# fudan-zvg/NeRF-LiDAR

Measured on AMD Instinct MI355X. Metric: LiDAR rays/sec @128 samples/ray, 8x256 MLP; depth L1 vs reference, higher is better.
Workload: dtype f32 (sampling, hash grid) + split-bf16 x3 MFMA (density/semantic/intensity) + bf16 MFMA (view MLP); 1 GPU; C2: nuScenes 32-beam sweep, 32x1024 rays per sweep, samples (64,64,128), 8x256 NerfMLP + semantic + intensity heads, full-size fp32 hash tables; azimuth_columns_total=1024, parallelism=azimuth-sector x1, hip_graph_replay=False, weights=seeded synthetic (white-noise tables, x1500 density gain), sweep_origins=moving: step i renders sweep i mod 64 (pre-uploaded ray batches), gather_bytes_per_ray=1347584

## Files before the change

nerf-lidar_amd/csrc/nlr_sample.hip:

```cpp
#include "nlr_kernels.h"

struct ResampleParams {
    const float *prev_sdist;
    const float *prev_weights;
    uint32_t n_prev;
    float dilation;
    float anneal, pad;
    uint32_t S;
    const float *u;
    const float *jitter;
    float max_jitter;
    const float *near, *far;
    float lam, lam1, c_fwd, inv_exp;
    uint32_t N;
    float *sdist, *tdist;
};

__device__ __forceinline__ float nlr_warp_fwd(float x, float lam, float lam1, float c_fwd) {
    return c_fwd * (powf((x * 2.0f) / lam1 + 1.0f, lam) - 1.0f);
}
__device__ __forceinline__ float nlr_warp_inv(float y, float lam, float lam1, float inv_exp) {
    return ((powf(((y * lam) / lam1 + 1.0f) + NLR_EPS, inv_exp) - 1.0f) * lam1) / 2.0f;
}

__global__ void __launch_bounds__(64) nlr_resample_kernel(ResampleParams P) {
    extern __shared__ __align__(16) float lds[];
    const uint32_t ray = blockIdx.x;
    const int lane = threadIdx.x;
    const uint32_t n = P.n_prev;
    const bool dilate = (n > 0) && (P.dilation > 0.0f);

    float *tt;
    float *ww;
    uint32_t m;
    float *scratch;

    if (n == 0) {
        tt = lds;
        ww = lds + 2;
        if (lane == 0) {
            tt[0] = 0.0f;
            tt[1] = 1.0f;
            ww[0] = 1.0f;
        }
        m = 1;
        scratch = lds + 4;
    } else {
        float *t = lds;
        float *p = t + (n + 1);
        const float *ps = P.prev_sdist + (size_t)ray * (n + 1);
        const float *pw = P.prev_weights + (size_t)ray * n;
        for (uint32_t i = lane; i <= n; i += 64) t[i] = ps[i];
        for (uint32_t i = lane; i < n; i += 64) p[i] = pw[i];
        __syncthreads();
        if (!dilate) {
            tt = t;
            ww = p;
            m = n;
            scratch = p + n;
        } else {
            float *U = p + n;
            float *W = U + (3 * n + 2);
            float *Mx = W + 3 * n;
            const float d = P.dilation;
            for (uint32_t j = lane; j < n; j += 64) p[j] = p[j] / fmaxf(t[j + 1] - t[j], NLR_EPS);
            auto count = [&](uint32_t len, auto pred) {
                uint32_t lo = 0, hi = len;
                while (lo < hi) {
                    const uint32_t mid = (lo + hi) >> 1;
                    if (pred(mid)) lo = mid + 1; else hi = mid;
                }
                return lo;
            };
            for (uint32_t i = lane; i <= 3 * n; i += 64) {
                float v;
                uint32_t r;
                if (i <= n) {
                    v = t[i];
                    r = i + count(n, [&](uint32_t q) { return (t[q] - d) < v; }) + count(n, [&](uint32_t q) { return (t[q + 1] + d) < v; });
                } else if (i <= 2 * n) {
                    const uint32_t o = i - (n + 1);
                    v = t[o] - d;
                    r = o + count(n + 1, [&](uint32_t q) { return t[q] <= v; }) + count(n, [&](uint32_t q) { return (t[q + 1] + d) < v; });
                } else {
                    const uint32_t o = i - (2 * n + 1);
                    v = t[o + 1] + d;
                    r = o + count(n + 1, [&](uint32_t q) { return t[q] <= v; }) + count(n, [&](uint32_t q) { return (t[q] - d) <= v; });
                }
                U[r] = fminf(fmaxf(v, 0.0f), 1.0f);
            }
            uint32_t LV = 1;
            while ((2u << (LV - 1)) <= n) ++LV;
            __syncthreads();
            for (uint32_t l = 1; l < LV; ++l) {
                const float *src = l == 1 ? p : Mx + (size_t)(l - 2) * n;
                float *dst = Mx + (size_t)(l - 1) * n;
                const uint32_t h2 = 1u << (l - 1);
                for (uint32_t j = lane; j < n; j += 64) {
                    const uint32_t j2 = j + h2 < n ? j + h2 : n - 1;
                    dst[j] = fmaxf(src[j], src[j2]);
                }
                __syncthreads();
            }
            float part = 0.0f;
            for (uint32_t k = lane; k < 3 * n; k += 64) {
                const float tk = U[k];
                const uint32_t j1 = count(n, [&](uint32_t q) { return (t[q] - d) <= tk; });
                const uint32_t j0 = count(n, [&](uint32_t q) { return (t[q + 1] + d) <= tk; });
                float best = 0.0f;
                if (j0 < j1) {
                    const uint32_t len = j1 - j0, l = 31u - (uint32_t)__clz((int)len);
                    const float *row = l == 0 ? p : Mx + (size_t)(l - 1) * n;
                    best = fmaxf(best, fmaxf(row[j0], row[j1 - (1u << l)]));
                }
                const float wk = best * (U[k + 1] - tk);
                W[k] = wk;
                part += wk;
            }
            const float tot = fmaxf(nlr_wave_sum(part), NLR_EPS);
            __syncthreads();
            for (uint32_t k = lane; k < 3 * n; k += 64) W[k] = W[k] / tot;
            __syncthreads();
            tt = U + 1;
            ww = W + 1;
            m = 3 * n - 2;
            scratch = Mx + (size_t)(LV - 1) * n;
        }
    }
    __syncthreads();

    float *cw = scratch;
    float *cen = cw + (m + 1);
    float mx = -INFINITY;
    for (uint32_t k = lane; k < m; k += 64) {
        const float lg = (tt[k + 1] > tt[k]) ? P.anneal * logf(ww[k] + P.pad) : -INFINITY;
        cw[k + 1] = lg;
        mx = fmaxf(mx, lg);
    }
    mx = nlr_wave_max(mx);
    float se = 0.0f;
    for (uint32_t k = lane; k < m; k += 64) {
        const float e = expf(cw[k + 1] - mx);
        cw[k + 1] = e;
        se += e;
    }
    se = nlr_wave_sum(se);
    __syncthreads();
    {
        const uint32_t per = (m + 63) / 64;
        const uint32_t b0 = lane * per;
        float run = 0.0f;
        for (uint32_t i = 0; i < per; ++i) {
            const uint32_t k = b0 + i;
            if (k < m) run += cw[k + 1] / se;
        }
        const float incl = nlr_wave_incl_scan_add(run, lane);
        float base = incl - run;
        float prevmax = nlr_wave_incl_scan_max(incl, lane);
        prevmax = __shfl_up(prevmax, 1, 64);
        if (lane == 0) prevmax = 0.0f;
        __syncthreads();
        float acc = base;
        float hi = prevmax;
        for (uint32_t i = 0; i < per; ++i) {
            const uint32_t k = b0 + i;
            if (k < m) {
                acc += cw[k + 1] / se;
                hi = fmaxf(hi, acc);
                cw[k + 1] = (k + 1 == m) ? 1.0f : fminf(hi, 1.0f);
            }
        }
        if (lane == 0) cw[0] = 0.0f;
    }
    __syncthreads();

    const float jit = P.jitter ? P.jitter[ray] * P.max_jitter : 0.0f;
    for (uint32_t k = lane; k < P.S; k += 64) {
        const float u = P.jitter ? P.u[k] + jit : P.u[k];
        uint32_t lo = 0, hi = m + 1;
        while (lo < hi) {
            const uint32_t mid = (lo + hi) >> 1;
            if (cw[mid] <= u) lo = mid + 1; else hi = mid;
        }
        const uint32_t i0 = lo > 0 ? (lo - 1 > m ? m : lo - 1) : 0;
        const uint32_t i1 = lo > m ? m : lo;
        const float x0 = cw[i0], x1 = cw[i1];
        float off = (u - x0) / (x1 - x0);
        if (off != off) off = 0.0f;
        off = fminf(fmaxf(off, 0.0f), 1.0f);
        cen[k] = tt[i0] + off * (tt[i1] - tt[i0]);
    }
    __syncthreads();

    const float nearv = P.near[ray], farv = P.far[ray];
    const float s_near = nlr_warp_fwd(nearv, P.lam, P.lam1, P.c_fwd);
    const float s_far = nlr_warp_fwd(farv, P.lam, P.lam1, P.c_fwd);
    float *so = P.sdist + (size_t)ray * (P.S + 1);
    float *to = P.tdist ? P.tdist + (size_t)ray * (P.S + 1) : nullptr;
    for (uint32_t k = lane; k <= P.S; k += 64) {
        float s;
        if (k == 0) {
            const float mid0 = (cen[1] + cen[0]) / 2.0f;
            s = fmaxf(2.0f * cen[0] - mid0, 0.0f);
        } else if (k == P.S) {
            const float midl = (cen[P.S - 1] + cen[P.S - 2]) / 2.0f;
            s = fminf(2.0f * cen[P.S - 1] - midl, 1.0f);
        } else {
            s = (cen[k] + cen[k - 1]) / 2.0f;
        }
        so[k] = s;
        if (to) to[k] = nlr_warp_inv(s * s_far + (1.0f - s) * s_near, P.lam, P.lam1, P.inv_exp);
    }
}

static void linspace_f32(float start, float end, uint32_t n, float *out) {
    if (n == 1) {
        out[0] = start;
        return;
    }
    const float step = (end - start) / (float)(n - 1);
    const uint32_t half = n / 2;
    for (uint32_t i = 0; i < n; ++i) out[i] = i < half ? start + step * (float)i : end - step * (float)(n - 1 - i);
}

extern "C" void nlr_sample_u(uint32_t n, int rand, float *u_host, float *max_jitter) {
    const double eps = (double)NLR_EPS;
    if (!rand) {
        const double pad = 1.0 / (2.0 * n);
        linspace_f32((float)pad, (float)(1.0 - pad - eps), n, u_host);
        if (max_jitter) *max_jitter = 0.0f;
    } else {
        const double u_max = eps + (1.0 - eps) / n;
        linspace_f32(0.0f, (float)(1.0 - u_max), n, u_host);
        if (max_jitter) *max_jitter = (float)((1.0 - u_max) / (n - 1) - eps);
    }
}

int nlr_launch_resample(const float *prev_sdist, const float *prev_weights, uint32_t n_prev, float dilation, float anneal,
                        float pad, uint32_t S, const float *u_dev, const float *jitter, float max_jitter, const float *near,
                        const float *far, float lam, uint32_t N, float *sdist, float *tdist, hipStream_t st) {
    NLR_CHECK_ARG(S >= 2, "num_samples must be > 1, is %u", S);
    NLR_CHECK_ARG(S <= 1024 && n_prev <= 512, "resample: S=%u / n_prev=%u beyond the LDS budget", S, n_prev);
    NLR_CHECK_ARG((n_prev == 0) || (prev_sdist && prev_weights), "resample: previous level tensors are NULL");
    ResampleParams P;
    memset(&P, 0, sizeof(P));
    P.prev_sdist = prev_sdist;
    P.prev_weights = prev_weights;
    P.n_prev = n_prev;
    P.dilation = dilation;
    P.anneal = anneal;
    P.pad = pad;
    P.S = S;
    P.u = u_dev;
    P.jitter = jitter;
    P.max_jitter = max_jitter;
    P.near = near;
    P.far = far;
    P.lam = lam;
    P.lam1 = fabsf(lam - 1.0f);
    P.c_fwd = (float)(fabs((double)lam - 1.0) / (double)lam);
    P.inv_exp = (float)(1.0 / (double)lam);
    P.N = N;
    P.sdist = sdist;
    P.tdist = tdist;
    const bool dilate = n_prev > 0 && dilation > 0.0f;
    size_t fl;
    uint32_t m;
    if (n_prev == 0) {
        fl = 4;
        m = 1;
    } else if (!dilate) {
        fl = 2 * (size_t)n_prev + 1;
        m = n_prev;
    } else {
        uint32_t lv = 1;
        while ((2u << (lv - 1)) <= n_prev) ++lv;
        fl = 2 * (size_t)n_prev + 1 + (3 * (size_t)n_prev + 2) + 3 * (size_t)n_prev + (size_t)(lv - 1) * n_prev;
        m = 3 * n_prev - 2;
    }
    fl += (m + 1) + S + 8;
    const size_t lds_bytes = fl * sizeof(float);
    NLR_CHECK_ARG(lds_bytes <= 64 * 1024, "resample: LDS need %zu B > 64 KiB", lds_bytes);
    hipLaunchKernelGGL(nlr_resample_kernel, dim3(N), dim3(64), lds_bytes, st, P);
    NLR_LAUNCH_CHECK("nlr_resample_kernel");
    return NLR_OK;
}

extern "C" int nlr_resample_level(const float *prev_sdist, const float *prev_weights, uint32_t n_prev, float dilation,
                                  float anneal, float resample_padding, uint32_t num_samples, const float *rand_jitter,
                                  const float *near, const float *far, float power_lambda, uint32_t N, float *sdist,
                                  float *tdist, void *stream) {
    NLR_CHECK_ARG(near && far && sdist, "resample_level: NULL tensor");
    if (N == 0) return NLR_OK;
    NLR_CHECK_ARG(num_samples >= 2 && num_samples <= 1024, "num_samples must be in [2,1024], is %u", num_samples);
    hipStream_t st = (hipStream_t)stream;
    float uh[1024], mj = 0.0f;
    nlr_sample_u(num_samples, rand_jitter != nullptr, uh, &mj);
    float *u_dev = nullptr;
    NLR_HIP(hipMallocAsync((void **)&u_dev, num_samples * sizeof(float), st));
    NLR_HIP(hipMemcpyAsync(u_dev, uh, num_samples * sizeof(float), hipMemcpyHostToDevice, st));
    NLR_HIP(hipStreamSynchronize(st));
    int rc = nlr_launch_resample(prev_sdist, prev_weights, n_prev, dilation, anneal, resample_padding, num_samples, u_dev,
                                 rand_jitter, mj, near, far, power_lambda, N, sdist, tdist, st);
    (void)hipFreeAsync(u_dev, st);
    return rc;
}
```

Measured before the change: 5.173 million rays/s.

## Replace per-element binary searches with chunked merge-style searches in resample kernel

The dilation merge-rank and max-query phases now give each lane a contiguous chunk and search two sorted lists at once. The first element of a chunk is searched in full, and the following elements narrow the bounds using the neighbouring lane's result via shuffles. Shifted boundary arrays are precomputed into LDS, the inverse-CDF sampling uses the same chunked search, and the first pass skips the softmax/scan when weights are uniform. It also computes the near/far warp in two lanes and broadcasts the result. The cost targeted is the many full-length LDS binary searches per element, at the price of more complex indexing, extra LDS scratch and load imbalance across lanes.

Result: faster. 5.346 million rays/s (median of 6 runs) (+3.3%).

```diff
diff --git a/nerf-lidar_amd/csrc/nlr_sample.hip b/nerf-lidar_amd/csrc/nlr_sample.hip
--- a/nerf-lidar_amd/csrc/nlr_sample.hip
+++ b/nerf-lidar_amd/csrc/nlr_sample.hip
@@ -23,6 +23,19 @@
     return ((powf(((y * lam) / lam1 + 1.0f) + NLR_EPS, inv_exp) - 1.0f) * lam1) / 2.0f;
 }
 
+__device__ __forceinline__ void nlr_count2(const float *l1, uint32_t &lo1, uint32_t hi1, bool eq1, const float *l2, uint32_t &lo2,
+                                           uint32_t hi2, bool eq2, float v) {
+    while (lo1 < hi1 || lo2 < hi2) {
+        const uint32_t m1 = (lo1 + hi1) >> 1, m2 = (lo2 + hi2) >> 1;
+        const float x1 = l1[m1], x2 = l2[m2];
+        const bool b1 = (x1 < v) | ((x1 == v) & eq1), b2 = (x2 < v) | ((x2 == v) & eq2);
+        lo1 = (b1 & (lo1 < hi1)) ? m1 + 1 : lo1;
+        hi1 = b1 ? hi1 : m1;
+        lo2 = (b2 & (lo2 < hi2)) ? m2 + 1 : lo2;
+        hi2 = b2 ? hi2 : m2;
+    }
+}
+
 __global__ void __launch_bounds__(64) nlr_resample_kernel(ResampleParams P) {
     extern __shared__ __align__(16) float lds[];
     const uint32_t ray = blockIdx.x;
@@ -34,6 +47,7 @@
     float *ww;
     uint32_t m;
     float *scratch;
+    bool uniform = false;
 
     if (n == 0) {
         tt = lds;
@@ -45,6 +59,8 @@
         }
         m = 1;
         scratch = lds + 4;
+        const float lg = P.anneal * logf(1.0f + P.pad);
+        uniform = (lg - lg) == 0.0f;
     } else {
         float *t = lds;
         float *p = t + (n + 1);
@@ -63,34 +79,43 @@
             float *W = U + (3 * n + 2);
             float *Mx = W + 3 * n;
             const float d = P.dilation;
-            for (uint32_t j = lane; j < n; j += 64) p[j] = p[j] / fmaxf(t[j + 1] - t[j], NLR_EPS);
-            auto count = [&](uint32_t len, auto pred) {
-                uint32_t lo = 0, hi = len;
-                while (lo < hi) {
-                    const uint32_t mid = (lo + hi) >> 1;
-                    if (pred(mid)) lo = mid + 1; else hi = mid;
-                }
-                return lo;
-            };
-            for (uint32_t i = lane; i <= 3 * n; i += 64) {
-                float v;
-                uint32_t r;
-                if (i <= n) {
-                    v = t[i];
-                    r = i + count(n, [&](uint32_t q) { return (t[q] - d) < v; }) + count(n, [&](uint32_t q) { return (t[q + 1] + d) < v; });
-                } else if (i <= 2 * n) {
-                    const uint32_t o = i - (n + 1);
-                    v = t[o] - d;
-                    r = o + count(n + 1, [&](uint32_t q) { return t[q] <= v; }) + count(n, [&](uint32_t q) { return (t[q + 1] + d) < v; });
-                } else {
-                    const uint32_t o = i - (2 * n + 1);
-                    v = t[o + 1] + d;
-                    r = o + count(n + 1, [&](uint32_t q) { return t[q] <= v; }) + count(n, [&](uint32_t q) { return (t[q] - d) <= v; });
-                }
-                U[r] = fminf(fmaxf(v, 0.0f), 1.0f);
-            }
             uint32_t LV = 1;
             while ((2u << (LV - 1)) <= n) ++LV;
+            float *t0 = Mx + (size_t)(LV - 1) * n;
+            float *t1 = t0 + n;
+            for (uint32_t j = lane; j < n; j += 64) {
+                const float a = t[j], b = t[j + 1];
+                p[j] = p[j] / fmaxf(b - a, NLR_EPS);
+                t0[j] = a - d;
+                t1[j] = b + d;
+            }
+            __syncthreads();
+            {
+                uint32_t per = (3 * n + 1 + 63) / 64;
+                while ((n + per) / per + 2 * ((n + per - 1) / per) > 64) ++per;
+                const uint32_t LA = (n + per) / per, LB = (n + per - 1) / per;
+                const uint32_t kind = (uint32_t)lane < LA ? 0u : ((uint32_t)lane < LA + LB ? 1u : 2u);
+                const float *own = kind == 0 ? t : (kind == 1 ? t0 : t1);
+                const float *l1 = kind == 0 ? t0 : t, *l2 = kind == 2 ? t0 : t1;
+                const uint32_t own_len = kind == 0 ? n + 1 : n, len1 = kind == 0 ? n : n + 1, len2 = n;
+                const bool eq1 = kind != 0, eq2 = kind == 2;
+                const uint32_t first_lane = kind == 0 ? 0u : (kind == 1 ? LA : LA + LB);
+                const uint32_t o0 = ((uint32_t)lane - first_lane) * per;
+                const uint32_t o1 = o0 + per < own_len ? o0 + per : own_len;
+                const bool act = o0 < own_len;
+                uint32_t c1 = 0, c2 = 0;
+                float v = act ? own[o0] : 0.0f;
+                nlr_count2(l1, c1, act ? len1 : 0u, eq1, l2, c2, act ? len2 : 0u, eq2, v);
+                const uint32_t n1 = __shfl_down(c1, 1, 64), n2 = __shfl_down(c2, 1, 64);
+                const bool next_same = ((uint32_t)lane + 1 - first_lane) * per < own_len && lane < 63;
+                const uint32_t up1 = next_same ? n1 : len1, up2 = next_same ? n2 : len2;
+                if (act) U[o0 + c1 + c2] = fminf(fmaxf(v, 0.0f), 1.0f);
+                for (uint32_t o = o0 + 1; o < o1; ++o) {
+                    v = own[o];
+                    nlr_count2(l1, c1, up1, eq1, l2, c2, up2, eq2, v);
+                    U[o + c1 + c2] = fminf(fmaxf(v, 0.0f), 1.0f);
+                }
+            }
             __syncthreads();
             for (uint32_t l = 1; l < LV; ++l) {
                 const float *src = l == 1 ? p : Mx + (size_t)(l - 2) * n;
@@ -102,21 +127,36 @@
                 }
                 __syncthreads();
             }
+            {
+                const uint32_t per = (3 * n + 63) / 64;
+                const uint32_t k0 = (uint32_t)lane * per, k1 = k0 + per < 3 * n ? k0 + per : 3 * n;
+                float tk = 0.0f;
+                const auto emit = [&](uint32_t k, uint32_t j0, uint32_t j1) {
+                    float best = 0.0f;
+                    if (j0 < j1) {
+                        const uint32_t len = j1 - j0, l = 31u - (uint32_t)__clz((int)len);
+                        const float *row = l == 0 ? p : Mx + (size_t)(l - 1) * n;
+                        best = fmaxf(best, fmaxf(row[j0], row[j1 - (1u << l)]));
+                    }
+                    W[k] = best * (U[k + 1] - tk);
+                };
+                const bool act = k0 < 3 * n;
+                uint32_t j1 = 0, j0 = 0;
+                if (act) tk = U[k0];
+                nlr_count2(t0, j1, act ? n : 0u, true, t1, j0, act ? n : 0u, true, tk);
+                const uint32_t nj1 = __shfl_down(j1, 1, 64), nj0 = __shfl_down(j0, 1, 64);
+                const bool next_act = ((uint32_t)lane + 1) * per < 3 * n && lane < 63;
+                const uint32_t up1 = next_act ? nj1 : n, up0 = next_act ? nj0 : n;
+                if (act) emit(k0, j0, j1);
+                for (uint32_t k = k0 + 1; k < k1; ++k) {
+                    tk = U[k];
+                    nlr_count2(t0, j1, up1, true, t1, j0, up0, true, tk);
+                    emit(k, j0, j1);
+                }
+            }
+            __syncthreads();
             float part = 0.0f;
-            for (uint32_t k = lane; k < 3 * n; k += 64) {
-                const float tk = U[k];
-                const uint32_t j1 = count(n, [&](uint32_t q) { return (t[q] - d) <= tk; });
-                const uint32_t j0 = count(n, [&](uint32_t q) { return (t[q + 1] + d) <= tk; });
-                float best = 0.0f;
-                if (j0 < j1) {
-                    const uint32_t len = j1 - j0, l = 31u - (uint32_t)__clz((int)len);
-                    const float *row = l == 0 ? p : Mx + (size_t)(l - 1) * n;
-                    best = fmaxf(best, fmaxf(row[j0], row[j1 - (1u << l)]));
-                }
-                const float wk = best * (U[k + 1] - tk);
-                W[k] = wk;
-                part += wk;
-            }
+            for (uint32_t k = lane; k < 3 * n; k += 64) part += W[k];
             const float tot = fmaxf(nlr_wave_sum(part), NLR_EPS);
             __syncthreads();
             for (uint32_t k = lane; k < 3 * n; k += 64) W[k] = W[k] / tot;
@@ -131,70 +171,93 @@
 
     float *cw = scratch;
     float *cen = cw + (m + 1);
-    float mx = -INFINITY;
-    for (uint32_t k = lane; k < m; k += 64) {
-        const float lg = (tt[k + 1] > tt[k]) ? P.anneal * logf(ww[k] + P.pad) : -INFINITY;
-        cw[k + 1] = lg;
-        mx = fmaxf(mx, lg);
-    }
-    mx = nlr_wave_max(mx);
-    float se = 0.0f;
-    for (uint32_t k = lane; k < m; k += 64) {
-        const float e = expf(cw[k + 1] - mx);
-        cw[k + 1] = e;
-        se += e;
-    }
-    se = nlr_wave_sum(se);
+    if (uniform) {
+        if (lane == 0) {
+            cw[0] = 0.0f;
+            cw[1] = 1.0f;
+        }
+    } else {
+        float mx = -INFINITY;
+        for (uint32_t k = lane; k < m; k += 64) {
+            const float lg = (tt[k + 1] > tt[k]) ? P.anneal * logf(ww[k] + P.pad) : -INFINITY;
+            cw[k + 1] = lg;
+            mx = fmaxf(mx, lg);
+        }
+        mx = nlr_wave_max(mx);
+        float se = 0.0f;
+        for (uint32_t k = lane; k < m; k += 64) {
+            const float e = expf(cw[k + 1] - mx);
+            cw[k + 1] = e;
+            se += e;
+        }
+        se = nlr_wave_sum(se);
+        __syncthreads();
+        {
+            const uint32_t per = (m + 63) / 64;
+            const uint32_t b0 = lane * per;
+            float run = 0.0f;
+            for (uint32_t i = 0; i < per; ++i) {
+                const uint32_t k = b0 + i;
+                if (k < m) run += cw[k + 1] / se;
+            }
+            const float incl = nlr_wave_incl_scan_add(run, lane);
+            float base = incl - run;
+            float prevmax = nlr_wave_incl_scan_max(incl, lane);
+            prevmax = __shfl_up(prevmax, 1, 64);
+            if (lane == 0) prevmax = 0.0f;
+            __syncthreads();
+            float acc = base;
+            float hi = prevmax;
+            for (uint32_t i = 0; i < per; ++i) {
+                const uint32_t k = b0 + i;
+                if (k < m) {
+                    acc += cw[k + 1] / se;
+                    hi = fmaxf(hi, acc);
+                    cw[k + 1] = (k + 1 == m) ? 1.0f : fminf(hi, 1.0f);
+                }
+            }
+            if (lane == 0) cw[0] = 0.0f;
+        }
+    }
     __syncthreads();
+
+    const float jit = P.jitter ? P.jitter[ray] * P.max_jitter : 0.0f;
     {
-        const uint32_t per = (m + 63) / 64;
-        const uint32_t b0 = lane * per;
-        float run = 0.0f;
-        for (uint32_t i = 0; i < per; ++i) {
-            const uint32_t k = b0 + i;
-            if (k < m) run += cw[k + 1] / se;
-        }
-        const float incl = nlr_wave_incl_scan_add(run, lane);
-        float base = incl - run;
-        float prevmax = nlr_wave_incl_scan_max(incl, lane);
-        prevmax = __shfl_up(prevmax, 1, 64);
-        if (lane == 0) prevmax = 0.0f;
-        __syncthreads();
-        float acc = base;
-        float hi = prevmax;
-        for (uint32_t i = 0; i < per; ++i) {
-            const uint32_t k = b0 + i;
-            if (k < m) {
-                acc += cw[k + 1] / se;
-                hi = fmaxf(hi, acc);
-                cw[k + 1] = (k + 1 == m) ? 1.0f : fminf(hi, 1.0f);
-            }
-        }
-        if (lane == 0) cw[0] = 0.0f;
+        const uint32_t per = (P.S + 63) / 64;
+        const uint32_t k0 = (uint32_t)lane * per, k1 = k0 + per < P.S ? k0 + per : P.S;
+        const auto emit = [&](uint32_t k, float u, uint32_t lo) {
+            const uint32_t i0 = lo > 0 ? (lo - 1 > m ? m : lo - 1) : 0;
+            const uint32_t i1 = lo > m ? m : lo;
+            const float x0 = cw[i0], x1 = cw[i1];
+            float off = (u - x0) / (x1 - x0);
+            if (off != off) off = 0.0f;
+            off = fminf(fmaxf(off, 0.0f), 1.0f);
+            cen[k] = tt[i0] + off * (tt[i1] - tt[i0]);
+        };
+        const auto search = [&](float u, uint32_t lo, uint32_t hi) {
+            while (lo < hi) {
+                const uint32_t mid = (lo + hi) >> 1;
+                if (cw[mid] <= u) lo = mid + 1; else hi = mid;
+            }
+            return lo;
+        };
+        const bool act = k0 < P.S;
+        float u = 0.0f;
+        if (act) u = P.jitter ? P.u[k0] + jit : P.u[k0];
+        uint32_t lo = search(u, 0, act ? m + 1 : 0u);
+        const uint32_t nlo = __shfl_down(lo, 1, 64);
+        const uint32_t up = (((uint32_t)lane + 1) * per < P.S && lane < 63) ? nlo : m + 1;
+        if (act) emit(k0, u, lo);
+        for (uint32_t k = k0 + 1; k < k1; ++k) {
+            u = P.jitter ? P.u[k] + jit : P.u[k];
+            lo = search(u, lo, up);
+            emit(k, u, lo);
+        }
     }
     __syncthreads();
 
-    const float jit = P.jitter ? P.jitter[ray] * P.max_jitter : 0.0f;
-    for (uint32_t k = lane; k < P.S; k += 64) {
-        const float u = P.jitter ? P.u[k] + jit : P.u[k];
-        uint32_t lo = 0, hi = m + 1;
-        while (lo < hi) {
-            const uint32_t mid = (lo + hi) >> 1;
-            if (cw[mid] <= u) lo = mid + 1; else hi = mid;
-        }
-        const uint32_t i0 = lo > 0 ? (lo - 1 > m ? m : lo - 1) : 0;
-        const uint32_t i1 = lo > m ? m : lo;
-        const float x0 = cw[i0], x1 = cw[i1];
-        float off = (u - x0) / (x1 - x0);
-        if (off != off) off = 0.0f;
-        off = fminf(fmaxf(off, 0.0f), 1.0f);
-        cen[k] = tt[i0] + off * (tt[i1] - tt[i0]);
-    }
-    __syncthreads();
-
-    const float nearv = P.near[ray], farv = P.far[ray];
-    const float s_near = nlr_warp_fwd(nearv, P.lam, P.lam1, P.c_fwd);
-    const float s_far = nlr_warp_fwd(farv, P.lam, P.lam1, P.c_fwd);
+    const float s_end = nlr_warp_fwd((lane & 1) ? P.far[ray] : P.near[ray], P.lam, P.lam1, P.c_fwd);
+    const float s_near = __shfl(s_end, 0, 64), s_far = __shfl(s_end, 1, 64);
     float *so = P.sdist + (size_t)ray * (P.S + 1);
     float *to = P.tdist ? P.tdist + (size_t)ray * (P.S + 1) : nullptr;
     for (uint32_t k = lane; k <= P.S; k += 64) {
```
